# talmolab/sleap

Hardware: NVIDIA H100
Metric: frames/sec (1024x1024 bottom-up UNet+PAF) (higher is better)
Workload: dtype f16

## Files before the change

sleap_b200/csrc/sb_conv_tc.cu:

```cuda
#include <cuda.h>

#include <algorithm>

#include "sb_model.h"

namespace {

constexpr int TW = 16, TH = 8;
constexpr int MAX_GROUPS = 7, MAX_TAPS = 7;
constexpr size_t kMaxDynSmem = 225 * 1024;

struct TcTap { int row_off, w_tap; };
struct TcGroup { int dx, n_taps; TcTap taps[MAX_TAPS]; };

struct TcParams {
  int H, W;
  int tiles_x;
  int n_chunks, KC;
  int n_groups;
  TcGroup groups[MAX_GROUPS];
  int dy0, box_rows;
  int N, Cout;
  void* out;
  int out_f32, out_H, out_W, out_Ctot, out_coff;
// ... 5 lines not shown
  void* pool_out;
  int pool_H, pool_W, pool_Ctot, pool_coff;
  const void* res;
  int res_Ctot, res_coff;
  int a_slot_bytes, b_slot_bytes, n_a_slots, n_b_slots;
  int a_tx_bytes, b_tx_bytes;
  int layout_type;
  int row_bytes;
  int epi_mode;
  int skip_out;
  int split;
  int pdl_trigger;
  int n_tiles, batch;
  const void* in;
  int in_Ctot, in_C;
};

#include "sb_tc_prims.cuh"

__device__ __forceinline__ void stage_params(const TcParams& P, float* s_par, int n0) {
  for (int i = threadIdx.x; i < P.N; i += blockDim.x) {
    const int co = n0 + i;
    const bool ok = co < P.Cout;
    s_par[i] = (ok && P.bias) ? P.bias[co] : 0.f;
    s_par[P.N + i] = (ok && P.bn_scale) ? P.bn_scale[co] : 1.f;
    s_par[2 * P.N + i] = (ok && P.bn_shift) ? P.bn_shift[co] : 0.f;
  }
}

template <int TWC = 0>
// ... 535 lines not shown
    }
  }
}

template <int N>
__device__ __forceinline__ void frag_rows_store(uint32_t (&hv)[N / 4], __half* po, size_t row_step, bool ok0, bool ok1, int t) {
  constexpr int NJ = N / 8;
#pragma unroll
  for (int c0 = 0; c0 < 2 * NJ; c0 += 4) {
    quad_transpose(hv[c0], hv[c0 + 1], hv[c0 + 2], hv[c0 + 3], t);
    const int c = c0 + t, r = c / NJ, j = c % NJ;
    if (r ? ok1 : ok0) *reinterpret_cast<uint4*>(po + r * row_step + 8 * j) = make_uint4(hv[c0], hv[c0 + 1], hv[c0 + 2], hv[c0 + 3]);
  }
}

template <int N>
__device__ __forceinline__ void halo_block_epilogue(const TcParams& P, const float (&acc)[N / 2], uint32_t s_bias, int n0, int b,
                                                    int y, int x, int g, int t, float lo) {
  constexpr int NJ = N / 8;
  uint32_t hv[2 * NJ];
  frag_rows_f16<N>(acc, s_bias, t, lo, hv);
  if (P.pool_out != nullptr) {
    constexpr int NJ4 = (NJ + 3) / 4 * 4;
    uint32_t pv[NJ4];
#pragma unroll
    for (int j = 0; j < NJ4; ++j) {
      if (j < NJ) {
        const uint32_t m0 = hmax2_u32(hv[j], __shfl_xor_sync(0xffffffffu, hv[j], 4));
        const uint32_t m1 = hmax2_u32(hv[NJ + j], __shfl_xor_sync(0xffffffffu, hv[NJ + j], 4));
        pv[j] = hmax2_u32(m0, m1);
      } else {
        pv[j] = 0u;
      }
    }
    __half* pp = reinterpret_cast<__half*>(P.pool_out) + (((size_t)b * P.pool_H + (y >> 1)) * P.pool_W + (x >> 1)) * P.pool_Ctot +
                 P.pool_coff + n0;
    const bool st = (g & 1) == 0 && y < P.H && x < P.W;
#pragma unroll
    for (int c0 = 0; c0 < NJ4; c0 += 4) {
      quad_transpose(pv[c0], pv[c0 + 1], pv[c0 + 2], pv[c0 + 3], t);
      if (st && c0 + t < NJ) *reinterpret_cast<uint4*>(pp + 8 * (c0 + t)) = make_uint4(pv[c0], pv[c0 + 1], pv[c0 + 2], pv[c0 + 3]);
    }
  }
  if (!P.skip_out) {
    __half* po = reinterpret_cast<__half*>(P.out) + (((size_t)b * P.out_H + y) * P.out_W + x) * P.out_Ctot + P.out_coff + n0;
    frag_rows_store<N>(hv, po, (size_t)P.out_W * P.out_Ctot, y < P.H && x < P.W, y + 1 < P.H && x < P.W, t);
  }
}

template <int KSTEPS, int N>
__global__ void __launch_bounds__(kHaloThreads, 1) k_conv_wg_h(const __grid_constant__ CUtensorMap mapA,
                                                               const __grid_constant__ CUtensorMap mapB,
                                                               const __grid_constant__ TcParams P) {
  constexpr int BY = halo_by(N, 16 * KSTEPS), NB = 2 * BY;
  constexpr int NP = 2 * KSTEPS;
  constexpr int PH = 8 * BY + 2, PW = kHaloCols, PLANE = halo_plane(N, 16 * KSTEPS), SLOT = NP * PLANE;
  constexpr int kLoaders = kHaloThreads - kConsumerThreads;
  extern __shared__ __align__(1024) uint8_t smem_raw[];
  uint8_t* base = reinterpret_cast<uint8_t*>((reinterpret_cast<uintptr_t>(smem_raw) + 1023) & ~(uintptr_t)1023);
  uint8_t* bank = base;
  uint8_t* ring = bank + 9 * (size_t)P.b_slot_bytes;
  uint64_t* full = reinterpret_cast<uint64_t*>(ring + (size_t)P.n_a_slots * SLOT);
  uint64_t* empty = full + P.n_a_slots;
  uint64_t* fullB = empty + P.n_a_slots;
  float* s_bias = reinterpret_cast<float*>(fullB + 1);

  const int warp = threadIdx.x >> 5, lane = threadIdx.x & 31;
  const int tiles_x = (P.W + 15) / 16, n_tiles = tiles_x * ((P.H + 8 * BY - 1) / (8 * BY));
  const int n_work = n_tiles * P.batch;
  for (int i = threadIdx.x; i < N; i += blockDim.x) s_bias[i] = (P.bias && i < P.Cout) ? P.bias[i] : 0.f;
  if (threadIdx.x == 0) {
    for (int i = 0; i < P.n_a_slots; ++i) { mbar_init(smem_u32(full + i), kLoaders); mbar_init(smem_u32(empty + i), 4); }
    mbar_init(smem_u32(fullB), 1);
    asm volatile("fence.mbarrier_init.release.cluster;" ::: "memory");
    asm volatile("prefetch.tensormap [%0];" ::"l"(&mapB) : "memory");
  }
  __syncthreads();

  if (warp < kLoaders / 32) {
    if (threadIdx.x == 0) {
      mbar_expect_tx(smem_u32(fullB), (uint32_t)(9 * P.b_tx_bytes));
      for (int kx = 0; kx < 3; ++kx)
        for (int ky = 0; ky < 3; ++ky)
          tma_load_3d(smem_u32(bank + (size_t)(kx * 3 + ky) * P.b_slot_bytes), &mapB, smem_u32(fullB), 0, 0, ky * 3 + kx);
    }
// ... 40 lines not shown
          }
        }
    wgmma_commit();
#pragma unroll
    for (int bk = 0; bk < NB; ++bk) wgmma_reg_fence(acc[bk]);
    wgmma_wait<0>();
#pragma unroll
    for (int bk = 0; bk < NB; ++bk) wgmma_reg_fence(acc[bk]);
    __syncwarp();
    if (lane == 0) mbar_arrive(smem_u32(empty + s));

    const int tile = w % n_tiles, b = w / n_tiles;
    const int x0 = (tile % tiles_x) * 16, y0 = (tile / tiles_x) * (8 * BY);
#pragma unroll
    for (int bk = 0; bk < NB; ++bk)
      halo_block_epilogue<N>(P, acc[bk], smem_u32(s_bias), 0, b, y0 + 8 * (bk >> 1) + 2 * q, x0 + 8 * (bk & 1) + g, g, t, lo);
  }
}

constexpr int kWideThreads = 384;
constexpr int kWidePatchLoaders = 96;
constexpr int wide_by(int n) { return n <= 64 ? 4 : 2; }
constexpr int wide_plane(int n) { return (8 * wide_by(n) + 2) * kHaloCols * 16; }

template <int N>
__global__ void __launch_bounds__(kWideThreads, 1) k_conv_wg_hw(const __grid_constant__ CUtensorMap mapA,
                                                                const __grid_constant__ CUtensorMap mapB,
                                                                const __grid_constant__ TcParams P) {
  constexpr int BY = wide_by(N), NP = 8, PH = 8 * BY + 2, PW = kHaloCols, PLANE = wide_plane(N), SLOT = NP * PLANE;
  constexpr int WSLOT = N * 128;
  extern __shared__ __align__(1024) uint8_t smem_raw[];
  uint8_t* base = reinterpret_cast<uint8_t*>((reinterpret_cast<uintptr_t>(smem_raw) + 1023) & ~(uintptr_t)1023);
  uint8_t* wring = base;
  uint8_t* pring = wring + (size_t)P.n_b_slots * WSLOT;
  uint64_t* pfull = reinterpret_cast<uint64_t*>(pring + (size_t)P.n_a_slots * SLOT);
  uint64_t* pempty = pfull + P.n_a_slots;
  uint64_t* wfull = pempty + P.n_a_slots;
  uint64_t* wempty = wfull + P.n_b_slots;
  float* s_bias = reinterpret_cast<float*>(wempty + P.n_b_slots);

  const int warp = threadIdx.x >> 5, lane = threadIdx.x & 31;
  const int tiles_x = (P.W + 15) / 16, n_pt = tiles_x * ((P.H + 8 * BY - 1) / (8 * BY));
  const int n_nt = P.Cout / N, n_work = n_nt * n_pt * P.batch;
  for (int i = threadIdx.x; i < P.Cout; i += blockDim.x) s_bias[i] = P.bias ? P.bias[i] : 0.f;
  if (threadIdx.x == 0) {
    for (int i = 0; i < P.n_a_slots; ++i) { mbar_init(smem_u32(pfull + i), kWidePatchLoaders); mbar_init(smem_u32(pempty + i), 8); }
    for (int i = 0; i < P.n_b_slots; ++i) { mbar_init(smem_u32(wfull + i), 1); mbar_init(smem_u32(wempty + i), 8); }
    asm volatile("fence.mbarrier_init.release.cluster;" ::: "memory");
    asm volatile("prefetch.tensormap [%0];" ::"l"(&mapB) : "memory");
  }
  __syncthreads();

  if (warp < 4) {
    setmaxnreg_dec<56>();
    if (warp != 1) {
      griddep_wait();
      const int pid = (warp == 0 ? 0 : 32 * (warp - 1)) + lane;
      for (int i = 0, w = blockIdx.x; w < n_work; w += gridDim.x) {
        if (w + (int)gridDim.x >= n_work) griddep_launch();
// ... 67 lines not shown
          rel_p = (kx == 2 && ky == 2) ? ps : -1;
          if (++ws == P.n_b_slots) { ws = 0; wph ^= 1; }
        }
      if (++ps == P.n_a_slots) { ps = 0; pph ^= 1; }
    }
    wgmma_wait<0>();
#pragma unroll
    for (int i = 0; i < BY; ++i) wgmma_reg_fence(acc[i]);
    __syncwarp();
    if (lane == 0) { mbar_arrive(smem_u32(wempty + rel_w)); mbar_arrive(smem_u32(pempty + rel_p)); }

    const int n0 = (w % n_nt) * N, pt = (w / n_nt) % n_pt, b = w / (n_nt * n_pt);
    const int x0 = (pt % tiles_x) * 16, y0 = (pt / tiles_x) * (8 * BY) + cw * (BY / 2) * 8;
#pragma unroll
    for (int i = 0; i < BY; ++i)
      halo_block_epilogue<N>(P, acc[i], smem_u32(s_bias + n0), n0, b, y0 + 8 * (i >> 1) + 2 * q, x0 + 8 * (i & 1) + g, g, t, lo);
  }
}

constexpr int kTconvBoxRows = 17;
constexpr int kTconvBox = kTconvBoxRows * 16 * 128;
struct TcPhases {
  int n_groups[4], dy0[4], oy_add[4], ox_add[4];
  TcGroup groups[4][2];
};

__device__ __forceinline__ int tconv_item(int r) {
  const int G = gridDim.x;
  return r * G + ((r & 1) ? G - 1 - (int)blockIdx.x : (int)blockIdx.x);
}

// ... 295 lines not shown
  dim3 grid;
  TcForm forms[kForms];
  int form;
};

}

struct SbConvTcPlan {
  std::vector<TcLaunch> launches;
  const void* head = nullptr;
  __half* w16 = nullptr;
  int Cout_pad = 0;
  bool pool_fused = false;
  bool out_dead = false;
  bool res_fused = false;
  std::vector<TcLaunch> plain_launches;
};

static CUtensorMapSwizzle swz_for(int KC) {
  return KC == 64 ? CU_TENSOR_MAP_SWIZZLE_128B : (KC == 32 ? CU_TENSOR_MAP_SWIZZLE_64B : CU_TENSOR_MAP_SWIZZLE_32B);
}

static bool tc_eligible(const SbModel* m, const SbOp& op) {
  if (getenv("SB_DISABLE_TC")) return false;
  if (op.kind() != SB_OPK_CONV && op.kind() != SB_OPK_TCONV) return false;
  const int Cin = op.in_C();
  if (!(Cin >= 16 && Cin % 8 == 0)) return false;
  if (op.kind() == SB_OPK_CONV && !((op.k() == 1 || op.k() == 3 || op.k() == 5 || op.k() == 7) && op.stride() == 1) &&
      !(op.k() == 1 && op.stride() == 2))
    return false;
// ... 32 lines not shown
  static const void* const kernels[kForms][8] = {
      {(const void*)k_conv_wg<KS, 16>, (const void*)k_conv_wg<KS, 32>, (const void*)k_conv_wg<KS, 48>,
       (const void*)k_conv_wg<KS, 64>, (const void*)k_conv_wg<KS, 96>, (const void*)k_conv_wg<KS, 128>,
       (const void*)k_conv_wg<KS, 192>, (const void*)k_conv_wg<KS, 256>},
      {(const void*)k_conv_wg_p<KS, 16>, (const void*)k_conv_wg_p<KS, 32>, (const void*)k_conv_wg_p<KS, 48>,
       (const void*)k_conv_wg_p<KS, 64>, (const void*)k_conv_wg_p<KS, 96>, (const void*)k_conv_wg_p<KS, 128>, nullptr, nullptr},
      {(const void*)k_conv_wg_h<KS, 16>, (const void*)k_conv_wg_h<KS, 32>, (const void*)k_conv_wg_h<KS, 48>,
       (const void*)k_conv_wg_h<KS, 64>, nullptr, nullptr, nullptr, nullptr},
      {nullptr, (const void*)k_conv_wg_hw<32>, (const void*)k_conv_wg_hw<48>, (const void*)k_conv_wg_hw<64>,
       (const void*)k_conv_wg_hw<96>, (const void*)k_conv_wg_hw<128>, nullptr, nullptr},
      {nullptr, (const void*)k_tconv_wg_hw<32>, (const void*)k_tconv_wg_hw<48>, (const void*)k_tconv_wg_hw<64>,
       (const void*)k_tconv_wg_hw<96>, (const void*)k_tconv_wg_hw<128>, nullptr, nullptr}};
  return form >= 3 && KS != 4 ? nullptr : kernels[form][ni];
}

static const void* form_kernel(int form, int KC, int N) {
  const int ni = (int)(std::find(std::begin(kWgN), std::end(kWgN), N) - std::begin(kWgN));
  if (ni == 8) return nullptr;
  return KC == 16 ? form_kernel_ks<1>(form, ni) : (KC == 32 ? form_kernel_ks<2>(form, ni) : form_kernel_ks<4>(form, ni));
}

static size_t conv_smem(const TcParams& P, int n_a, int n_b) {
  return (size_t)n_a * P.a_slot_bytes + (size_t)n_b * P.b_slot_bytes + (size_t)128 * (stage_cols(P.N) + 4) * sizeof(float) +
         1024  + (size_t)(2 * n_a + 2 * n_b) * 8 + 16 + 3 * 256 * sizeof(float);
}

static size_t conv_smem_resident(const TcParams& P, int n_a, int bank) {
  return (size_t)n_a * P.a_slot_bytes + (size_t)bank * P.b_slot_bytes + (size_t)128 * (stage_cols(P.N) + 4) * sizeof(float) +
         1024  + (size_t)(2 * n_a + 1) * 8 + 16 + 3 * (size_t)P.N * sizeof(float);
}

static size_t conv_smem_halo(const TcParams& P, int n_a) {
  return 1024  + (size_t)9 * P.b_slot_bytes + (size_t)n_a * (P.KC / 8) * halo_plane(P.N, P.KC) + (size_t)(2 * n_a + 1) * 8 +
         (size_t)P.N * sizeof(float);
}

static void fit_weight_ring(TcForm& F, int n_a, size_t a_slot) {
  for (int nb = 8; nb >= 4 && !F.ok; --nb) {
    const size_t smem = 1024  + (size_t)nb * F.P.N * 128 + (size_t)n_a * a_slot + (size_t)(2 * n_a + 2 * nb) * 8 +
                        (size_t)F.P.Cout * sizeof(float);
    if (smem <= kMaxDynSmem) { F.ok = 1; F.P.n_a_slots = n_a; F.P.n_b_slots = nb; F.smem = smem; }
  }
}

static void fit_ctas(sb_handle_s* h, TcForm& F, int f) {
  if (!F.ok) return;
  int nb = 0;
  if (cudaOccupancyMaxActiveBlocksPerMultiprocessor(&nb, form_kernel(f, F.P.KC, F.P.N), F.threads, F.smem) != cudaSuccess || nb < 1) {
    cudaGetLastError();
    F.ok = 0;
    return;
  }
  F.max_ctas = nb * h->sm_count;
}

static bool halo_shape(const TcParams& P) {
  if (P.epi_mode != 1 || P.res != nullptr || P.n_groups != 3 || P.dy0 != -1 || P.box_rows != TH + 2 || P.oy_mul != 1 ||
      P.oy_add != 0 || P.ox_mul != 1 || P.ox_add != 0)
    return false;
  for (int g = 0; g < 3; ++g) {
    if (P.groups[g].dx != g - 1 || P.groups[g].n_taps != 3) return false;
    for (int ky = 0; ky < 3; ++ky)
      if (P.groups[g].taps[ky].row_off != ky || P.groups[g].taps[ky].w_tap != 3 * ky + g) return false;
  }
  return true;
}

static bool halo_eligible(const TcLaunch& L) {
  const TcParams& P = L.forms[0].P;
  return L.grid.y == 1 && P.n_chunks == 1 && P.N <= 64 && halo_shape(P);
}

static int wide_n(const TcParams& P) { return std::min(P.N, 128); }
static bool wide_eligible(const TcParams& P) { return P.KC == 64 && P.Cout % wide_n(P) == 0 && halo_shape(P); }

static void setup_forms(sb_handle_s* h, TcLaunch& L, int total_steps) {
  const TcParams& P = L.forms[0].P;
  L.form = 0;
  for (int f = 1; f < kForms; ++f) {
    L.forms[f] = L.forms[0];
    L.forms[f].ok = 0;
  }
  if (TcForm& F = L.forms[3]; form_kernel(3, P.KC, wide_n(P)) && wide_eligible(P)) {
    F.threads = kWideThreads;
    F.P.N = wide_n(P);
    fit_weight_ring(F, 2, (size_t)8 * wide_plane(F.P.N));
    const int by = wide_by(F.P.N);
    F.n_items = (P.Cout / F.P.N) * ((P.W + 15) / 16) * ((P.H + 8 * by - 1) / (8 * by));
    fit_ctas(h, F, 3);
  }
  if (TcForm& F = L.forms[2]; form_kernel(2, P.KC, P.N) && halo_eligible(L)) {
    F.threads = kHaloThreads;
    for (int na = 8; na >= 4 && !F.ok; --na)
      if (conv_smem_halo(P, na) <= kMaxDynSmem) { F.ok = 1; F.P.n_a_slots = na; F.P.n_b_slots = 9; F.smem = conv_smem_halo(P, na); }
    const int by = halo_by(P.N, P.KC);
    F.n_items = ((P.W + 15) / 16) * ((P.H + 8 * by - 1) / (8 * by));
    fit_ctas(h, F, 2);
  }
  TcForm& F = L.forms[1];
  if (!form_kernel(1, P.KC, P.N) || L.grid.y != 1) return;
  const int bank = P.n_chunks * total_steps;
  for (size_t budget : {(size_t)113 * 1024, kMaxDynSmem}) {
    for (int na = 4; na >= 2 && !F.ok; --na)
      if (conv_smem_resident(P, na, bank) <= budget) { F.ok = 1; F.P.n_a_slots = na; F.P.n_b_slots = bank; F.smem = conv_smem_resident(P, na, bank); }
    if (F.ok) break;
  }
  F.n_items = P.n_tiles;
  fit_ctas(h, F, 1);
}
// ... 208 lines not shown
         (size_t)plan->Cout_pad * (op.in_C() + 8) * 2 <= 160 * 1024 && head_shape(op).n_ring >= 2;
}

static const void* head_kernel(int nt, int kch) {
#define SB_HEAD_CASE(NT)                                                                                                 \
  case NT:                                                                                                               \
    return kch == 16 ? (const void*)k_head_1x1<NT, 16> : kch == 32 ? (const void*)k_head_1x1<NT, 32>                     \
         : kch == 64 ? (const void*)k_head_1x1<NT, 64> : (const void*)k_head_1x1<NT, 128>;
  switch (nt) {
    SB_HEAD_CASE(1) SB_HEAD_CASE(2) SB_HEAD_CASE(3) SB_HEAD_CASE(4)
    default: return nullptr;
  }
#undef SB_HEAD_CASE
}

int sb_conv_tc_prepare(sb_handle_s* h, SbModel* m) {
  m->tc_plans.assign(m->ops.size(), nullptr);
  if (m->precision == 1) return 0;
  const bool split = m->precision == 2;
  static bool attr_set = false;
  if (!attr_set) {
    for (int f = 0; f < kForms; ++f)
      for (int kc : {16, 32, 64})
        for (int n : kWgN)
          if (const void* k = form_kernel(f, kc, n))
            SB_CUDA(h, cudaFuncSetAttribute(k, cudaFuncAttributeMaxDynamicSharedMemorySize, (int)kMaxDynSmem));
    attr_set = true;
  }
  for (size_t oi = 0; oi < m->ops.size(); ++oi) {
    const SbOp& op = m->ops[oi];
    if (!tc_eligible(m, op)) continue;
    const int Cin = op.in_C(), Cout = op.out_C(), k = op.k(), taps = k * k;
    SbConvTcPlan* plan = new SbConvTcPlan();
    int cp = (Cout + 15) / 16 * 16;
    if (cp > 256) cp = (cp + 255) / 256 * 256;
    plan->Cout_pad = cp;
    std::vector<__half> w16((size_t)taps * cp * Cin, __float2half(0.f));
    const float* w = m->weights_host.data() + op.w_off();
    for (int t = 0; t < taps; ++t)
      for (int ci = 0; ci < Cin; ++ci)
        for (int co = 0; co < Cout; ++co)
// ... 58 lines not shown
            ++ng;
          }
          rc = make_launch(h, m, op, plan, ng, g, a == 0 ? -1 : 0, extra, 9, 2, a, 2, bx);
        }
    }
    if (!rc && op.kind() == SB_OPK_TCONV) rc = setup_tconv_form(h, m, op, plan);
    if (rc) { cudaFree(plan->w16); delete plan; return rc; }
    m->tc_plans[oi] = plan;
    if (head_kernel_ok(m, op, plan)) {
      const HeadShape hs = head_shape(op);
      plan->head = head_kernel(hs.nt, hs.kch);
      SB_CUDA(h, cudaFuncSetAttribute(plan->head, cudaFuncAttributeMaxDynamicSharedMemorySize, (int)kHeadSmem));
    }
    if (op.kind() == SB_OPK_CONV && op.pool_buf() >= 0 && oi + 1 < m->ops.size() &&
        m->ops[oi + 1].kind() == SB_OPK_POOL && (m->ops[oi + 1].flags() & SB_OPF_FUSED_POOL))
      if (plan->launches[0].forms[0].P.pool_out != nullptr) {
        plan->pool_fused = true;
        bool read = false;
        for (size_t oj = 0; oj < m->ops.size() && !read; ++oj) {
          if (oj == oi || oj == oi + 1) continue;
          const SbOp& o2 = m->ops[oj];
          if (o2.kind() == SB_OPK_PREPROCESS) continue;
          const int ext = split ? 3 * Cout : Cout;
          const bool overl_in = o2.in_buf() == op.out_buf() && o2.in_coff() < op.out_coff() + ext && op.out_coff() < o2.in_coff() + o2.in_C();
          const bool overl_in2 = o2.kind() == SB_OPK_ADD && o2.in2_buf() == op.out_buf() && o2.in2_coff() < op.out_coff() + ext &&
                                 op.out_coff() < o2.in2_coff() + o2.in_C();
          read = overl_in || overl_in2;
        }
        plan->out_dead = !read;
      }
  }
  return 0;
}

bool sb_pdl_on() {
  static int v = -1;
  if (v < 0) v = getenv("SB_DISABLE_PDL") ? 0 : 1;
  return v != 0;
}

static void launch_form(const TcLaunch& L, int B, cudaStream_t stream, int skip_out) {
  const TcForm& F = L.forms[L.form];
  TcParams P = F.P;
  P.skip_out = skip_out;
  dim3 grid(std::min(F.n_items * B, F.max_ctas));
  size_t smem = F.smem;
  if (L.form == 0) {
    grid = dim3(L.grid.x, L.grid.y, B);
    P.pdl_trigger = (sb_pdl_on() && smem >= 114 * 1024) ? 1 : 0;
    if (P.pdl_trigger) smem = std::max(smem, kMaxDynSmem);
  } else {
    P.batch = B;
  }
  void* args[4] = {const_cast<CUtensorMap*>(&F.mapA), const_cast<CUtensorMap*>(&F.mapB), &P, const_cast<TcPhases*>(&F.Q)};
  sb_launch_pdl(form_kernel(L.form, P.KC, P.N), grid, dim3(F.threads), smem, stream, args);
}

static int tc_launch(sb_handle_s* h, const std::vector<TcLaunch>& launches, int B, int skip_out) {
  for (const TcLaunch& L : launches) {
    launch_form(L, B, h->stream, skip_out);
    SB_CHECK_LAUNCH(h);
    if (L.form == kTconvForm) break;
  }
  return 0;
}

int sb_time_min(sb_handle_s* h, const char* what, float& best, const std::function<int()>& run) {
  cudaEvent_t e0, e1;
  SB_CUDA(h, cudaEventCreate(&e0));
  SB_CUDA(h, cudaEventCreate(&e1));
// ... 2 lines not shown
  for (int rep = 0; rep < 4 && !rc; ++rep) {
    cudaEventRecord(e0, h->stream);
    if ((rc = run())) break;
    cudaEventRecord(e1, h->stream);
    if (cudaError_t e = cudaStreamSynchronize(h->stream); e != cudaSuccess)
      rc = sb_fail(h, SB_ERR_CUDA, "autotune launch (%s) failed: %s", what, cudaGetErrorString(e));
    float ms = 0.f;
    cudaEventElapsedTime(&ms, e0, e1);
    if (rep > 0) best = std::min(best, ms);
  }
  cudaEventDestroy(e0);
  cudaEventDestroy(e1);
  return rc;
}

int sb_conv_tc_autotune(sb_handle_s* h, SbModel* m) {
  char what[64];
  const bool dbg = getenv("SB_DEBUG") != nullptr;
  const char* fvar = getenv("SB_FORCE_VARIANT");
  const int force = fvar ? atoi(fvar) : -1;
  static const char* const form_name[kForms] = {"streaming", "resident", "halo", "wide", "tconv-fused"};
  for (size_t oi = 0; oi < m->tc_plans.size(); ++oi) {
    SbConvTcPlan* plan = m->tc_plans[oi];
    if (!plan || plan->head) continue;
    for (std::vector<TcLaunch>* list : {&plan->launches, &plan->plain_launches})
      for (size_t li = 0; li < list->size(); ++li) {
        TcLaunch& L = (*list)[li];
        float best[kTconvForm];
        int pick = 0;
        for (int f = 0; f < kTconvForm; ++f) {
          best[f] = 1e30f;
          if (!L.forms[f].ok) continue;
          L.form = f;
          snprintf(what, sizeof what, "op %zu, %s form", oi, form_name[f]);
          const int rc = sb_time_min(h, what, best[f], [&] {
            launch_form(L, m->B, h->stream, plan->out_dead && list == &plan->launches);
            return 0;
          });
          if (rc) return rc;
          if (best[f] < best[pick]) pick = f;
        }
        L.form = (force >= 0 && force < kTconvForm && L.forms[force].ok) ? force : pick;
        if (dbg) {
          fprintf(stderr, "[sb_conv_tc] op %zu launch %zu%s:", oi, li, list == &plan->launches ? "" : " (own output)");
          for (int f = 0; f < kTconvForm; ++f)
            if (L.forms[f].ok) fprintf(stderr, " %s %.1f us", form_name[f], best[f] * 1e3f);
          fprintf(stderr, " -> %s\n", form_name[L.form]);
        }
      }
  }
  for (size_t oi = 0; oi < m->tc_plans.size(); ++oi) {
    SbConvTcPlan* plan = m->tc_plans[oi];
    if (!plan || plan->launches.empty() || !plan->launches[0].forms[kTconvForm].ok) continue;
    TcLaunch& L0 = plan->launches[0];
    const int phase_form = L0.form;
    float best[2];
    for (int f = 0; f < 2; ++f) {
      L0.form = f ? kTconvForm : phase_form;
      snprintf(what, sizeof what, "op %zu, %s", oi, f ? "fused tconv" : "tconv phases");
      if (const int rc = sb_time_min(h, what, best[f], [&] { return tc_launch(h, plan->launches, m->B, 0); })) return rc;
    }
    L0.form = (force >= 0 ? force == kTconvForm : best[1] < best[0]) ? kTconvForm : phase_form;
    if (dbg)
      fprintf(stderr, "[sb_conv_tc] op %zu launches (4 tconv phases) %.1f us, fused k_tconv_wg_hw %.1f us -> %s\n", oi, best[0] * 1e3f,
              best[1] * 1e3f, L0.form == kTconvForm ? "tconv-fused" : "phases");
  }
  return 0;
}

static SbLaunchFn head_entry(const SbModel* m, const SbOp& op, const SbConvTcPlan* plan, bool log) {
  const SbBuffer& ib = m->buffers[op.in_buf()];
  const SbBuffer& ob = m->buffers[op.out_buf()];
  const HeadShape hs = head_shape(op);
  if (log && getenv("SB_DEBUG"))
    fprintf(stderr, "[sb_conv_tc] head k_head_1x1: Cin %d Cout %d NT %d KCH %d n_ring %d smem %zu\n", op.in_C(), op.out_C(), hs.nt,
            hs.kch, hs.n_ring, hs.smem);
  const void* kern = plan->head;
  const __half* in = (const __half*)ib.dev;
  const __half* w = plan->w16;
  const float* bias = op.b_off() >= 0 ? m->weights_dev + op.b_off() : nullptr;
// ... 10 lines not shown
    return 0;
  };
}

SbTcEntry sb_conv_tc_entry(const SbModel* m, int op_index, bool all_stores) {
  const SbConvTcPlan* plan = m->tc_plans[op_index];
  SbTcEntry e;
  if (plan->head) {
    e.run = head_entry(m, m->ops[op_index], plan, !all_stores);
    return e;
  }
  const bool res = plan->res_fused && !all_stores;
  const int skip = plan->out_dead && !all_stores;
  const std::vector<TcLaunch>* launches = plan->res_fused && all_stores ? &plan->plain_launches : &plan->launches;
  e.run = [launches, skip](sb_handle_s* h, const void*, int, int B) { return tc_launch(h, *launches, B, skip); };
  if (plan->pool_fused || res) e.absorbs = op_index + 1;
  e.elides_out = skip || res;
  return e;
}
```

sleap_b200/csrc/sb_model.cu:

```cuda
#include <algorithm>

#include "sb_common.cuh"
#include "sb_kernels_direct.cuh"
#include "sb_model.h"

using namespace sbd;

namespace {

template <typename T> T* buf_ptr(const SbBuffer& b) { return (T*)b.dev; }

size_t elem_size(const SbModel* m, const SbBuffer& b) { return (b.f32 || m->precision == 1) ? 4 : 2; }

int grid_for(size_t total, int sm) {
  size_t g = (total + 255) / 256;
  size_t cap = (size_t)sm * 16;
  return (int)std::max<size_t>(1, std::min(g, cap));
}

int build_programs(sb_handle_s* h, SbModel* m);

}

void sb_global_scratch_free(SbGlobalScratch& g) {
// ... 353 lines not shown
        SB_CHECK_LAUNCH(h);
        return 0;
      };
      return 0;
    default:
      return sb_fail(h, SB_ERR_INVALID, "unknown op kind %d", op.kind());
  }
}

int build_programs(sb_handle_s* h, SbModel* m) {
  const size_t n = m->ops.size();
  m->op_kind.assign(n, 0);
  for (size_t oi = 0; oi < n; ++oi)
    if (m->ops[oi].kind() == SB_OPK_CONV || m->ops[oi].kind() == SB_OPK_TCONV) m->op_kind[oi] = m->tc_plans[oi] ? 1 : 2;
  m->buf_elided.assign(m->buffers.size(), 0);
  for (int all_stores = 0; all_stores < 2; ++all_stores) {
    m->prog[all_stores].assign(n, nullptr);
    std::vector<char> taken(n, 0);
    sb_entry_build(m, all_stores, taken);
    for (size_t oi = 0; oi < n; ++oi) {
      if (taken[oi]) continue;
      if (m->tc_plans[oi]) {
        const SbTcEntry e = sb_conv_tc_entry(m, (int)oi, all_stores);
        m->prog[all_stores][oi] = e.run;
        if (e.absorbs >= 0) taken[e.absorbs] = 1;
        if (e.elides_out) m->buf_elided[m->ops[oi].out_buf()] = 1;
        continue;
      }
      const int rc = m->precision == 1 ? op_entry_t<float>(h, m, m->ops[oi], m->prog[all_stores][oi])
                                       : op_entry_t<__half>(h, m, m->ops[oi], m->prog[all_stores][oi]);
      if (rc) return rc;
    }
  }
  return 0;
}

int run_program(sb_handle_s* h, SbModel* m, const std::vector<SbLaunchFn>& prog, const void* frames_dev, int frames_are_u8, int B) {
  cudaStream_t s = h->stream;
  for (size_t oi = 0; oi < prog.size(); ++oi) {
    if (!m->prof_events.empty()) cudaEventRecord(m->prof_events[oi], s);
// ... 106 lines not shown
  if (out_n) *out_n = n;
  m->fwd_n = 0;
  if (enable && m->fwd_events.empty()) {
    m->fwd_events.resize(2 * 1024);
    for (auto& e : m->fwd_events) SB_CUDA(h, cudaEventCreate(&e));
  }
  m->fwd_timing = enable != 0;
  return SB_OK;
}

}


static int post_guard_op(const SbModel* m, int b0, int b1, int b2) {
  if (getenv("SB_DISABLE_POST_OVERLAP")) return -1;
  for (size_t i = 0; i < m->ops.size(); ++i) {
    const int ob = m->ops[i].out_buf();
    if (ob == b0 || ob == b1 || (b2 >= 0 && ob == b2)) return (int)i;
  }
  return -1;
}

static size_t record_width(const SbModel* m) {
  if (m->chain == SB_CHAIN_GLOBAL) return (size_t)m->buffers[m->gl.cms_buffer].C * 3;
  return m->chain == SB_CHAIN_CLASS ? sb_class_record_width(m->mc.n_classes, m->mc.n_nodes) : sb_record_width(m->bu.max_instances, m->bu.n_nodes);
}

struct SbMap {
  const float* dev;
  int H, W, C;
};
static SbMap head_map(const SbModel* m, int buf) {
  const SbBuffer& b = m->buffers[buf];
  return {(const float*)b.dev, b.H, b.W, b.C};
}
// ... 639 lines not shown
```

sleap_b200/csrc/sb_model.h:

```cpp
#pragma once
#include <functional>
#include <vector>

#include "sb_common.cuh"

enum {
  SB_OPK_BUFFER = 0,
  SB_OPK_CONV = 1,
  SB_OPK_TCONV = 2,
  SB_OPK_POOL = 3,
  SB_OPK_UPSAMPLE = 4,
  SB_OPK_ADD = 5,
  SB_OPK_PREPROCESS = 6,
  SB_OPK_COPY = 7,
};
enum { SB_OPF_RELU = 1, SB_OPF_BN = 2, SB_OPF_BILINEAR = 8, SB_OPF_FUSED_POOL = 16, SB_OPF_EXPLICIT_PAD = 32,
       SB_OPF_FUSED_ADD = 64, SB_OPF_RESIDUAL = 128 };
enum { SB_PRE_PLAIN = 0, SB_PRE_IMAGENET_CAFFE = 1, SB_PRE_IMAGENET_CAFFE_GRAY = 2 };

struct SbOp {
  int32_t w[SB_OP_WORDS];
  int kind() const { return w[0]; }
  int in_buf() const { return w[1]; }
  int in_coff() const { return w[2]; }
// ... 62 lines not shown
  int precision = 0;
  std::vector<SbOp> ops;
  std::vector<SbBuffer> buffers;
  std::vector<float> weights_host;
  float* weights_dev = nullptr;
  void* weights_tc_dev = nullptr;
  int64_t n_weights = 0;
  bool configured = false;
  int B = 0, Hin = 0, Win = 0, Cin = 0, Hres = 0, Wres = 0, Hnet = 0, Wnet = 0;
  size_t act_bytes = 0;
  void* frames_dev = nullptr;
  std::vector<SbConvTcPlan*> tc_plans;
  std::vector<SbLaunchFn> prog[2];
  std::vector<int> op_kind;
  std::vector<char> buf_elided;
  std::vector<cudaEvent_t> prof_events;
  std::vector<cudaEvent_t> fwd_events;
  int fwd_n = 0;
  bool fwd_timing = false;
  int chain = SB_CHAIN_NONE;
  unsigned chain_gen = 0;
  SbPostWs ws;
  sb_bottomup_params bu{};
  std::vector<int> bu_edges;
  sb_multiclass_params mc{};
  int guard_op = -1;
  void* frames_slot[2] = {nullptr, nullptr};
  float* stage_host[2] = {nullptr, nullptr};
  int slot_B[2] = {0, 0}, rec_B = 0;
  float* rec_host = nullptr;
// ... 23 lines not shown
bool sb_topdown_busy(const SbModel* m);

int sb_track_records_alloc(sb_handle_s* h, SbModel* m, int B, int I);

SbGatherDev sb_gather_dev(const SbModel* m, unsigned long long step);
void sb_gather_free(SbModel* m);
int sb_gather_queue_collect(sb_handle_s* h, SbModel* m, long long step, int B, float* host_dst, int* counts_dev, cudaStream_t s);
void sb_pipeline_slots_free(SbModel* m);
int sb_slot_upload(sb_handle_s* h, SbModel* m, const uint8_t* frames_host, int B, int slot);

int sb_conv_tc_prepare(sb_handle_s* h, SbModel* m);
int sb_conv_tc_autotune(sb_handle_s* h, SbModel* m);
void sb_conv_tc_release(SbModel* m);
struct SbTcEntry {
  SbLaunchFn run;
  int absorbs = -1;
  bool elides_out = false;
};
SbTcEntry sb_conv_tc_entry(const SbModel* m, int op_index, bool all_stores);
struct SbTcView {
  SbBuffer in;
  SbBuffer out;
  int Cout = 0, out_coff = 0;
  int R = 0, S = 0, dy0 = 0, dx0 = 0;
  const float *bias = nullptr, *bn_scale = nullptr, *bn_shift = nullptr;
  int relu = 0;
};
int sb_conv_tc_view_prepare(sb_handle_s* h, SbModel* m, int op_index, const SbTcView& v, const std::vector<float>& w);
void sb_conv_tc_drop(SbModel* m, int op_index);
int sb_time_min(sb_handle_s* h, const char* what, float& best, const std::function<int()>& run);

// ... 21 lines not shown
```

Measured before the change: 4244.

## Fuse 1x1 output head conv into preceding 3x3 conv epilogue

Adds an optional head path to the halo and wide wgmma conv kernels. The 1x1 head conv (confidence maps / PAFs) is computed in the epilogue with mma.sync on the f16 fragments already in registers, and f32 head outputs are written directly. This avoids a separate head kernel launch and a reread of the feature map. An autotune step times fused against separate execution and keeps the faster one. It also adds scheduling bookkeeping (run_by, a list of absorbed ops) so the post-processing overlap guard still works, at the cost of extra shared memory that may shrink the ring slots.

Measured after the change: 4264 (median of 6 runs). Within noise of the previous version (+0.5%).

```diff
diff --git a/sleap_b200/csrc/sb_conv_tc.cu b/sleap_b200/csrc/sb_conv_tc.cu
--- a/sleap_b200/csrc/sb_conv_tc.cu
+++ b/sleap_b200/csrc/sb_conv_tc.cu
@@ -43,6 +43,10 @@
   int n_tiles, batch;
   const void* in;
   int in_Ctot, in_C;
+  const __half* head_w;
+  const float* head_bias;
+  float* head_out;
+  int head_nt, head_Cout, head_Ctot, head_coff, head_relu;
 };
 
 #include "sb_tc_prims.cuh"
@@ -608,12 +612,73 @@
   }
 }
 
+constexpr int kHeadMaxNt = 4;
+__host__ __device__ constexpr size_t head_smem(int N, int nt) {
+  return nt ? 16 + (size_t)8 * nt * (N + 8) * 2 + (size_t)8 * nt * 4 : 0;
+}
+struct HeadSmem {
+  uint32_t w, bias;
+};
 template <int N>
+__device__ __forceinline__ HeadSmem stage_head(const TcParams& P, uint8_t* p) {
+  __half* s_w = reinterpret_cast<__half*>((reinterpret_cast<uintptr_t>(p) + 15) & ~(uintptr_t)15);
+  float* s_b = reinterpret_cast<float*>(s_w + 8 * P.head_nt * (N + 8));
+  for (int i = threadIdx.x; i < 8 * P.head_nt * (N / 8); i += blockDim.x) {
+    const int r = i / (N / 8), c8 = i % (N / 8);
+    *reinterpret_cast<uint4*>(s_w + r * (N + 8) + 8 * c8) = *reinterpret_cast<const uint4*>(P.head_w + (size_t)r * N + 8 * c8);
+  }
+  for (int i = threadIdx.x; i < 8 * P.head_nt; i += blockDim.x) s_b[i] = (i < P.head_Cout && P.head_bias) ? P.head_bias[i] : 0.f;
+  return HeadSmem{smem_u32(s_w), smem_u32(s_b)};
+}
+
+__device__ __forceinline__ uint32_t lds_u32(uint32_t saddr) {
+  uint32_t v;
+  asm("ld.shared.u32 %0, [%1];" : "=r"(v) : "r"(saddr));
+  return v;
+}
+
+template <int N>
+__device__ __forceinline__ void head_block(const TcParams& P, const HeadSmem& hs, const uint32_t (&hv)[N / 4], int b, int y, int x0,
+                                           int g, int t) {
+  constexpr int NJ = N / 8;
+  const int nt = P.head_nt, C = P.head_Cout, px = x0 + g;
+  const bool ok0 = px < P.W && y < P.H, ok1 = px < P.W && y + 1 < P.H;
+  float* o0 = P.head_out + (((size_t)b * P.H + y) * P.W + px) * P.head_Ctot + P.head_coff;
+  float* o1 = o0 + (size_t)P.W * P.head_Ctot;
+#pragma unroll(N >= 128 ? kHeadMaxNt : 1)
+  for (int n = 0; n < kHeadMaxNt; ++n) {
+    if (n >= nt) break;
+    float a0 = 0.f, a1 = 0.f, a2 = 0.f, a3 = 0.f;
+#pragma unroll
+    for (int s = 0; s < N / 16; ++s) {
+      const uint32_t wb = hs.w + 2u * (uint32_t)((8 * n + g) * (N + 8) + 16 * s + 2 * t);
+      asm volatile("mma.sync.aligned.m16n8k16.row.col.f32.f16.f16.f32 {%0, %1, %2, %3}, {%4, %5, %6, %7}, {%8, %9}, {%0, %1, %2, %3};"
+                   : "+f"(a0), "+f"(a1), "+f"(a2), "+f"(a3)
+                   : "r"(hv[2 * s]), "r"(hv[NJ + 2 * s]), "r"(hv[2 * s + 1]), "r"(hv[NJ + 2 * s + 1]), "r"(lds_u32(wb)),
+                     "r"(lds_u32(wb + 16u)));
+    }
+    const int c = 8 * n + 2 * t;
+    const float2 bb = lds_f2(hs.bias + 4u * c);
+    float v0 = a0 + bb.x, v1 = a1 + bb.y, v2 = a2 + bb.x, v3 = a3 + bb.y;
+    if (P.head_relu) { v0 = fmaxf(v0, 0.f); v1 = fmaxf(v1, 0.f); v2 = fmaxf(v2, 0.f); v3 = fmaxf(v3, 0.f); }
+    if (c < C) {
+      if (ok0) o0[c] = v0;
+      if (ok1) o1[c] = v2;
+    }
+    if (c + 1 < C) {
+      if (ok0) o0[c + 1] = v1;
+      if (ok1) o1[c + 1] = v3;
+    }
+  }
+}
+
+template <int N, bool HEAD>
 __device__ __forceinline__ void halo_block_epilogue(const TcParams& P, const float (&acc)[N / 2], uint32_t s_bias, int n0, int b,
-                                                    int y, int x, int g, int t, float lo) {
+                                                    int y, int x, int g, int t, float lo, const HeadSmem& hs) {
   constexpr int NJ = N / 8;
   uint32_t hv[2 * NJ];
   frag_rows_f16<N>(acc, s_bias, t, lo, hv);
+  if constexpr (HEAD) head_block<N>(P, hs, hv, b, y, x - g, g, t);
   if (P.pool_out != nullptr) {
     constexpr int NJ4 = (NJ + 3) / 4 * 4;
     uint32_t pv[NJ4];
@@ -642,7 +707,7 @@
   }
 }
 
-template <int KSTEPS, int N>
+template <int KSTEPS, int N, bool HEAD = false>
 __global__ void __launch_bounds__(kHaloThreads, 1) k_conv_wg_h(const __grid_constant__ CUtensorMap mapA,
                                                                const __grid_constant__ CUtensorMap mapB,
                                                                const __grid_constant__ TcParams P) {
@@ -663,6 +728,8 @@
   const int tiles_x = (P.W + 15) / 16, n_tiles = tiles_x * ((P.H + 8 * BY - 1) / (8 * BY));
   const int n_work = n_tiles * P.batch;
   for (int i = threadIdx.x; i < N; i += blockDim.x) s_bias[i] = (P.bias && i < P.Cout) ? P.bias[i] : 0.f;
+  HeadSmem hs{};
+  if constexpr (HEAD) hs = stage_head<N>(P, reinterpret_cast<uint8_t*>(s_bias + N));
   if (threadIdx.x == 0) {
     for (int i = 0; i < P.n_a_slots; ++i) { mbar_init(smem_u32(full + i), kLoaders); mbar_init(smem_u32(empty + i), 4); }
     mbar_init(smem_u32(fullB), 1);
@@ -733,7 +800,7 @@
     const int x0 = (tile % tiles_x) * 16, y0 = (tile / tiles_x) * (8 * BY);
 #pragma unroll
     for (int bk = 0; bk < NB; ++bk)
-      halo_block_epilogue<N>(P, acc[bk], smem_u32(s_bias), 0, b, y0 + 8 * (bk >> 1) + 2 * q, x0 + 8 * (bk & 1) + g, g, t, lo);
+      halo_block_epilogue<N, HEAD>(P, acc[bk], smem_u32(s_bias), 0, b, y0 + 8 * (bk >> 1) + 2 * q, x0 + 8 * (bk & 1) + g, g, t, lo, hs);
   }
 }
 
@@ -742,7 +809,7 @@
 constexpr int wide_by(int n) { return n <= 64 ? 4 : 2; }
 constexpr int wide_plane(int n) { return (8 * wide_by(n) + 2) * kHaloCols * 16; }
 
-template <int N>
+template <int N, bool HEAD = false>
 __global__ void __launch_bounds__(kWideThreads, 1) k_conv_wg_hw(const __grid_constant__ CUtensorMap mapA,
                                                                 const __grid_constant__ CUtensorMap mapB,
                                                                 const __grid_constant__ TcParams P) {
@@ -762,6 +829,8 @@
   const int tiles_x = (P.W + 15) / 16, n_pt = tiles_x * ((P.H + 8 * BY - 1) / (8 * BY));
   const int n_nt = P.Cout / N, n_work = n_nt * n_pt * P.batch;
   for (int i = threadIdx.x; i < P.Cout; i += blockDim.x) s_bias[i] = P.bias ? P.bias[i] : 0.f;
+  HeadSmem hs{};
+  if constexpr (HEAD) hs = stage_head<N>(P, reinterpret_cast<uint8_t*>(s_bias + P.Cout));
   if (threadIdx.x == 0) {
     for (int i = 0; i < P.n_a_slots; ++i) { mbar_init(smem_u32(pfull + i), kWidePatchLoaders); mbar_init(smem_u32(pempty + i), 8); }
     for (int i = 0; i < P.n_b_slots; ++i) { mbar_init(smem_u32(wfull + i), 1); mbar_init(smem_u32(wempty + i), 8); }
@@ -859,7 +928,7 @@
     const int x0 = (pt % tiles_x) * 16, y0 = (pt / tiles_x) * (8 * BY) + cw * (BY / 2) * 8;
 #pragma unroll
     for (int i = 0; i < BY; ++i)
-      halo_block_epilogue<N>(P, acc[i], smem_u32(s_bias + n0), n0, b, y0 + 8 * (i >> 1) + 2 * q, x0 + 8 * (i & 1) + g, g, t, lo);
+      halo_block_epilogue<N, HEAD>(P, acc[i], smem_u32(s_bias + n0), n0, b, y0 + 8 * (i >> 1) + 2 * q, x0 + 8 * (i & 1) + g, g, t, lo, hs);
   }
 }
 
@@ -1185,6 +1254,7 @@
   bool pool_fused = false;
   bool out_dead = false;
   bool res_fused = false;
+  int head_op = -1;
   std::vector<TcLaunch> plain_launches;
 };
 
@@ -1247,7 +1317,17 @@
   return form >= 3 && KS != 4 ? nullptr : kernels[form][ni];
 }
 
-static const void* form_kernel(int form, int KC, int N) {
+template <int KS>
+static const void* head_form_kernel_ks(int form, int N) {
+  if (form == 2) return N == 16 ? (const void*)k_conv_wg_h<KS, 16, true> : N == 32 ? (const void*)k_conv_wg_h<KS, 32, true>
+                      : N == 64 ? (const void*)k_conv_wg_h<KS, 64, true> : nullptr;
+  if (form == 3 && KS == 4) return N == 32 ? (const void*)k_conv_wg_hw<32, true> : N == 64 ? (const void*)k_conv_wg_hw<64, true>
+                                 : N == 128 ? (const void*)k_conv_wg_hw<128, true> : nullptr;
+  return nullptr;
+}
+
+static const void* form_kernel(int form, int KC, int N, bool head = false) {
+  if (head) return KC == 16 ? head_form_kernel_ks<1>(form, N) : (KC == 32 ? head_form_kernel_ks<2>(form, N) : head_form_kernel_ks<4>(form, N));
   const int ni = (int)(std::find(std::begin(kWgN), std::end(kWgN), N) - std::begin(kWgN));
   if (ni == 8) return nullptr;
   return KC == 16 ? form_kernel_ks<1>(form, ni) : (KC == 32 ? form_kernel_ks<2>(form, ni) : form_kernel_ks<4>(form, ni));
@@ -1265,13 +1345,13 @@
 
 static size_t conv_smem_halo(const TcParams& P, int n_a) {
   return 1024  + (size_t)9 * P.b_slot_bytes + (size_t)n_a * (P.KC / 8) * halo_plane(P.N, P.KC) + (size_t)(2 * n_a + 1) * 8 +
-         (size_t)P.N * sizeof(float);
+         (size_t)P.N * sizeof(float) + head_smem(P.N, P.head_nt);
 }
 
 static void fit_weight_ring(TcForm& F, int n_a, size_t a_slot) {
   for (int nb = 8; nb >= 4 && !F.ok; --nb) {
     const size_t smem = 1024  + (size_t)nb * F.P.N * 128 + (size_t)n_a * a_slot + (size_t)(2 * n_a + 2 * nb) * 8 +
-                        (size_t)F.P.Cout * sizeof(float);
+                        (size_t)F.P.Cout * sizeof(float) + head_smem(F.P.N, F.P.head_nt);
     if (smem <= kMaxDynSmem) { F.ok = 1; F.P.n_a_slots = n_a; F.P.n_b_slots = nb; F.smem = smem; }
   }
 }
@@ -1279,7 +1359,8 @@
 static void fit_ctas(sb_handle_s* h, TcForm& F, int f) {
   if (!F.ok) return;
   int nb = 0;
-  if (cudaOccupancyMaxActiveBlocksPerMultiprocessor(&nb, form_kernel(f, F.P.KC, F.P.N), F.threads, F.smem) != cudaSuccess || nb < 1) {
+  const void* k = form_kernel(f, F.P.KC, F.P.N, F.P.head_out != nullptr);
+  if (!k || cudaOccupancyMaxActiveBlocksPerMultiprocessor(&nb, k, F.threads, F.smem) != cudaSuccess || nb < 1) {
     cudaGetLastError();
     F.ok = 0;
     return;
@@ -1307,6 +1388,11 @@
 static int wide_n(const TcParams& P) { return std::min(P.N, 128); }
 static bool wide_eligible(const TcParams& P) { return P.KC == 64 && P.Cout % wide_n(P) == 0 && halo_shape(P); }
 
+static void fit_patch_ring(TcForm& F) {
+  for (int na = 8; na >= 4 && !F.ok; --na)
+    if (conv_smem_halo(F.P, na) <= kMaxDynSmem) { F.ok = 1; F.P.n_a_slots = na; F.P.n_b_slots = 9; F.smem = conv_smem_halo(F.P, na); }
+}
+
 static void setup_forms(sb_handle_s* h, TcLaunch& L, int total_steps) {
   const TcParams& P = L.forms[0].P;
   L.form = 0;
@@ -1324,8 +1410,7 @@
   }
   if (TcForm& F = L.forms[2]; form_kernel(2, P.KC, P.N) && halo_eligible(L)) {
     F.threads = kHaloThreads;
-    for (int na = 8; na >= 4 && !F.ok; --na)
-      if (conv_smem_halo(P, na) <= kMaxDynSmem) { F.ok = 1; F.P.n_a_slots = na; F.P.n_b_slots = 9; F.smem = conv_smem_halo(P, na); }
+    fit_patch_ring(F);
     const int by = halo_by(P.N, P.KC);
     F.n_items = ((P.W + 15) / 16) * ((P.H + 8 * by - 1) / (8 * by));
     fit_ctas(h, F, 2);
@@ -1564,17 +1649,59 @@
 #undef SB_HEAD_CASE
 }
 
+static int head_fusable(const SbModel* m, size_t oi) {
+  const SbOp& op = m->ops[oi];
+  const SbConvTcPlan* plan = m->tc_plans[oi];
+  if (getenv("SB_DISABLE_HEAD_FUSION") || m->precision == 2 || op.kind() != SB_OPK_CONV || plan->head || plan->launches.size() != 1)
+    return -1;
+  const TcLaunch& L = plan->launches[0];
+  bool form_ok = false;
+  for (int f : {2, 3})
+    form_ok |= L.forms[f].ok && L.forms[f].P.N == op.out_C() && L.forms[f].P.epi_mode == 1 && form_kernel(f, L.forms[f].P.KC, L.forms[f].P.N, true);
+  if (!form_ok) return -1;
+  for (size_t hj = oi + 1; hj < m->ops.size(); ++hj) {
+    const SbOp& hd = m->ops[hj];
+    if (m->tc_plans[hj] && m->tc_plans[hj]->head && hd.in_buf() == op.out_buf() && hd.in_coff() == op.out_coff() && hd.in_C() == op.out_C()) {
+      for (size_t oj = oi + 1; oj < hj; ++oj) {
+        const SbOp& o2 = m->ops[oj];
+        if (o2.out_buf() == hd.out_buf() || o2.in_buf() == hd.out_buf() || (o2.kind() == SB_OPK_ADD && o2.in2_buf() == hd.out_buf()) ||
+            m->buffers[o2.out_buf()].f32)
+          return -1;
+      }
+      return (int)hj;
+    }
+    if (hd.out_buf() == op.out_buf()) return -1;
+  }
+  return -1;
+}
+
+static bool out_read(const SbModel* m, size_t oi) {
+  const SbOp& op = m->ops[oi];
+  const SbConvTcPlan* plan = m->tc_plans[oi];
+  const int ext = m->precision == 2 ? 3 * op.out_C() : op.out_C();
+  for (size_t oj = 0; oj < m->ops.size(); ++oj) {
+    if (oj == oi || (plan->pool_fused && oj == oi + 1)) continue;
+    const SbOp& o2 = m->ops[oj];
+    if (o2.kind() == SB_OPK_PREPROCESS) continue;
+    const bool overl_in = o2.in_buf() == op.out_buf() && o2.in_coff() < op.out_coff() + ext && op.out_coff() < o2.in_coff() + o2.in_C();
+    const bool overl_in2 = o2.kind() == SB_OPK_ADD && o2.in2_buf() == op.out_buf() && o2.in2_coff() < op.out_coff() + ext &&
+                           op.out_coff() < o2.in2_coff() + o2.in_C();
+    if (overl_in || overl_in2) return true;
+  }
+  return false;
+}
+
 int sb_conv_tc_prepare(sb_handle_s* h, SbModel* m) {
   m->tc_plans.assign(m->ops.size(), nullptr);
   if (m->precision == 1) return 0;
-  const bool split = m->precision == 2;
   static bool attr_set = false;
   if (!attr_set) {
     for (int f = 0; f < kForms; ++f)
       for (int kc : {16, 32, 64})
         for (int n : kWgN)
-          if (const void* k = form_kernel(f, kc, n))
-            SB_CUDA(h, cudaFuncSetAttribute(k, cudaFuncAttributeMaxDynamicSharedMemorySize, (int)kMaxDynSmem));
+          for (bool head : {false, true})
+            if (const void* k = form_kernel(f, kc, n, head))
+              SB_CUDA(h, cudaFuncSetAttribute(k, cudaFuncAttributeMaxDynamicSharedMemorySize, (int)kMaxDynSmem));
     attr_set = true;
   }
   for (size_t oi = 0; oi < m->ops.size(); ++oi) {
@@ -1663,22 +1790,40 @@
     }
     if (op.kind() == SB_OPK_CONV && op.pool_buf() >= 0 && oi + 1 < m->ops.size() &&
         m->ops[oi + 1].kind() == SB_OPK_POOL && (m->ops[oi + 1].flags() & SB_OPF_FUSED_POOL))
-      if (plan->launches[0].forms[0].P.pool_out != nullptr) {
-        plan->pool_fused = true;
-        bool read = false;
-        for (size_t oj = 0; oj < m->ops.size() && !read; ++oj) {
-          if (oj == oi || oj == oi + 1) continue;
-          const SbOp& o2 = m->ops[oj];
-          if (o2.kind() == SB_OPK_PREPROCESS) continue;
-          const int ext = split ? 3 * Cout : Cout;
-          const bool overl_in = o2.in_buf() == op.out_buf() && o2.in_coff() < op.out_coff() + ext && op.out_coff() < o2.in_coff() + o2.in_C();
-          const bool overl_in2 = o2.kind() == SB_OPK_ADD && o2.in2_buf() == op.out_buf() && o2.in2_coff() < op.out_coff() + ext &&
-                                 op.out_coff() < o2.in2_coff() + o2.in_C();
-          read = overl_in || overl_in2;
-        }
-        plan->out_dead = !read;
-      }
-  }
+      plan->pool_fused = plan->launches[0].forms[0].P.pool_out != nullptr;
+  }
+  for (size_t oi = 0; oi < m->ops.size(); ++oi) {
+    SbConvTcPlan* plan = m->tc_plans[oi];
+    const int hj = plan ? head_fusable(m, oi) : -1;
+    if (hj < 0) continue;
+    const SbOp& hd = m->ops[hj];
+    const SbBuffer& hb = m->buffers[hd.out_buf()];
+    plan->plain_launches = plan->launches;
+    TcLaunch& L = plan->launches[0];
+    for (int f = 0; f < kForms; ++f) {
+      TcForm& F = L.forms[f];
+      const bool ok = (f == 2 || f == 3) && F.ok && F.P.N == m->ops[oi].out_C();
+      F.ok = 0;
+      if (!ok) continue;
+      TcParams& P = F.P;
+      P.head_w = m->tc_plans[hj]->w16;
+      P.head_bias = hd.b_off() >= 0 ? m->weights_dev + hd.b_off() : nullptr;
+      P.head_out = (float*)hb.dev;
+      P.head_nt = (hd.out_C() + 7) / 8; P.head_Cout = hd.out_C(); P.head_Ctot = hb.C; P.head_coff = hd.out_coff();
+      P.head_relu = (hd.flags() & SB_OPF_RELU) ? 1 : 0;
+      if (f == 2) fit_patch_ring(F);
+      else fit_weight_ring(F, 2, (size_t)8 * wide_plane(P.N));
+      fit_ctas(h, F, f);
+    }
+    if (L.forms[2].ok || L.forms[3].ok) {
+      plan->head_op = hj;
+    } else {
+      plan->launches = plan->plain_launches;
+      plan->plain_launches.clear();
+    }
+  }
+  for (size_t oi = 0; oi < m->ops.size(); ++oi)
+    if (SbConvTcPlan* plan = m->tc_plans[oi]; plan && plan->pool_fused) plan->out_dead = !out_read(m, oi);
   return 0;
 }
 
@@ -1702,7 +1847,7 @@
     P.batch = B;
   }
   void* args[4] = {const_cast<CUtensorMap*>(&F.mapA), const_cast<CUtensorMap*>(&F.mapB), &P, const_cast<TcPhases*>(&F.Q)};
-  sb_launch_pdl(form_kernel(L.form, P.KC, P.N), grid, dim3(F.threads), smem, stream, args);
+  sb_launch_pdl(form_kernel(L.form, P.KC, P.N, P.head_out != nullptr), grid, dim3(F.threads), smem, stream, args);
 }
 
 static int tc_launch(sb_handle_s* h, const std::vector<TcLaunch>& launches, int B, int skip_out) {
@@ -1735,6 +1880,8 @@
   return rc;
 }
 
+static SbLaunchFn head_entry(const SbModel* m, const SbOp& op, const SbConvTcPlan* plan, bool log);
+
 int sb_conv_tc_autotune(sb_handle_s* h, SbModel* m) {
   char what[64];
   const bool dbg = getenv("SB_DEBUG") != nullptr;
@@ -1744,7 +1891,9 @@
   for (size_t oi = 0; oi < m->tc_plans.size(); ++oi) {
     SbConvTcPlan* plan = m->tc_plans[oi];
     if (!plan || plan->head) continue;
-    for (std::vector<TcLaunch>* list : {&plan->launches, &plan->plain_launches})
+    const bool forced = force >= 0 && force < kTconvForm;
+    for (std::vector<TcLaunch>* list : {&plan->launches, &plan->plain_launches}) {
+      if (list == &plan->launches && plan->head_op >= 0 && forced && !(*list)[0].forms[force].ok) continue;
       for (size_t li = 0; li < list->size(); ++li) {
         TcLaunch& L = (*list)[li];
         float best[kTconvForm];
@@ -1769,6 +1918,7 @@
           fprintf(stderr, " -> %s\n", form_name[L.form]);
         }
       }
+    }
   }
   for (size_t oi = 0; oi < m->tc_plans.size(); ++oi) {
     SbConvTcPlan* plan = m->tc_plans[oi];
@@ -1785,6 +1935,44 @@
     if (dbg)
       fprintf(stderr, "[sb_conv_tc] op %zu launches (4 tconv phases) %.1f us, fused k_tconv_wg_hw %.1f us -> %s\n", oi, best[0] * 1e3f,
               best[1] * 1e3f, L0.form == kTconvForm ? "tconv-fused" : "phases");
+  }
+  for (size_t oi = 0; oi < m->tc_plans.size(); ++oi) {
+    SbConvTcPlan* plan = m->tc_plans[oi];
+    if (!plan || plan->head_op < 0) continue;
+    const TcLaunch &L = plan->launches[0], &L1 = plan->plain_launches[0];
+    bool fuse = false;
+    if (force >= 0 && force < kTconvForm) {
+      fuse = L.forms[force].ok != 0;
+      if (dbg)
+        fprintf(stderr, "[sb_conv_tc] op %zu + head op %d: SB_FORCE_VARIANT=%d%s%s -> %s\n", oi, plan->head_op, force,
+                fuse ? ", head-fused " : "", fuse ? form_name[L.form] : "", fuse ? "head-fused" : "separate");
+    } else {
+      const SbLaunchFn head = head_entry(m, m->ops[plan->head_op], m->tc_plans[plan->head_op], false);
+      float best[2];
+      snprintf(what, sizeof what, "op %zu, conv + head", oi);
+      if (const int rc = sb_time_min(h, what, best[0], [&] {
+            launch_form(L1, m->B, h->stream, 0);
+            return head(h, nullptr, 0, m->B);
+          }))
+        return rc;
+      snprintf(what, sizeof what, "op %zu, head-fused", oi);
+      if (const int rc = sb_time_min(h, what, best[1], [&] {
+            launch_form(L, m->B, h->stream, plan->out_dead);
+            return 0;
+          }))
+        return rc;
+      fuse = best[1] < best[0];
+      if (dbg)
+        fprintf(stderr, "[sb_conv_tc] op %zu + head op %d: %s + k_head_1x1 %.1f us, head-fused %s %.1f us (%d / %d ring slots, "
+                        "%d / %d without the head) -> %s\n", oi, plan->head_op, form_name[L1.form], best[0] * 1e3f, form_name[L.form],
+                best[1] * 1e3f, L.forms[L.form].P.n_a_slots, L.forms[L.form].P.n_b_slots, L1.forms[L.form].P.n_a_slots,
+                L1.forms[L.form].P.n_b_slots, fuse ? "head-fused" : "separate");
+    }
+    if (!fuse) {
+      plan->launches = plan->plain_launches;
+      plan->head_op = -1;
+    }
+    plan->plain_launches.clear();
   }
   return 0;
 }
@@ -1825,7 +2013,8 @@
   const int skip = plan->out_dead && !all_stores;
   const std::vector<TcLaunch>* launches = plan->res_fused && all_stores ? &plan->plain_launches : &plan->launches;
   e.run = [launches, skip](sb_handle_s* h, const void*, int, int B) { return tc_launch(h, *launches, B, skip); };
-  if (plan->pool_fused || res) e.absorbs = op_index + 1;
+  if (plan->pool_fused || res) e.absorbs.push_back(op_index + 1);
+  if (plan->head_op >= 0) e.absorbs.push_back(plan->head_op);
   e.elides_out = skip || res;
   return e;
 }
diff --git a/sleap_b200/csrc/sb_model.cu b/sleap_b200/csrc/sb_model.cu
--- a/sleap_b200/csrc/sb_model.cu
+++ b/sleap_b200/csrc/sb_model.cu
@@ -391,6 +391,8 @@
   for (size_t oi = 0; oi < n; ++oi)
     if (m->ops[oi].kind() == SB_OPK_CONV || m->ops[oi].kind() == SB_OPK_TCONV) m->op_kind[oi] = m->tc_plans[oi] ? 1 : 2;
   m->buf_elided.assign(m->buffers.size(), 0);
+  m->run_by.resize(n);
+  for (size_t oi = 0; oi < n; ++oi) m->run_by[oi] = (int)oi;
   for (int all_stores = 0; all_stores < 2; ++all_stores) {
     m->prog[all_stores].assign(n, nullptr);
     std::vector<char> taken(n, 0);
@@ -400,7 +402,10 @@
       if (m->tc_plans[oi]) {
         const SbTcEntry e = sb_conv_tc_entry(m, (int)oi, all_stores);
         m->prog[all_stores][oi] = e.run;
-        if (e.absorbs >= 0) taken[e.absorbs] = 1;
+        for (const int a : e.absorbs) {
+          taken[a] = 1;
+          if (!all_stores) m->run_by[a] = (int)oi;
+        }
         if (e.elides_out) m->buf_elided[m->ops[oi].out_buf()] = 1;
         continue;
       }
@@ -537,11 +542,12 @@
 
 static int post_guard_op(const SbModel* m, int b0, int b1, int b2) {
   if (getenv("SB_DISABLE_POST_OVERLAP")) return -1;
+  int guard = -1;
   for (size_t i = 0; i < m->ops.size(); ++i) {
     const int ob = m->ops[i].out_buf();
-    if (ob == b0 || ob == b1 || (b2 >= 0 && ob == b2)) return (int)i;
-  }
-  return -1;
+    if ((ob == b0 || ob == b1 || (b2 >= 0 && ob == b2)) && (guard < 0 || m->run_by[i] < guard)) guard = m->run_by[i];
+  }
+  return guard;
 }
 
 static size_t record_width(const SbModel* m) {
diff --git a/sleap_b200/csrc/sb_model.h b/sleap_b200/csrc/sb_model.h
--- a/sleap_b200/csrc/sb_model.h
+++ b/sleap_b200/csrc/sb_model.h
@@ -100,6 +100,7 @@
   std::vector<SbLaunchFn> prog[2];
   std::vector<int> op_kind;
   std::vector<char> buf_elided;
+  std::vector<int> run_by;
   std::vector<cudaEvent_t> prof_events;
   std::vector<cudaEvent_t> fwd_events;
   int fwd_n = 0;
@@ -153,7 +154,7 @@
 void sb_conv_tc_release(SbModel* m);
 struct SbTcEntry {
   SbLaunchFn run;
-  int absorbs = -1;
+  std::vector<int> absorbs;
   bool elides_out = false;
 };
 SbTcEntry sb_conv_tc_entry(const SbModel* m, int op_index, bool all_stores);
```
